# google-research/se3ds

Hardware: AMD Instinct MI355X
Metric: panoramas/sec (G+D train step) at 512x1024 RGB-D (higher is better)
Workload: dtype bf16; 1 GPU; configs/highres 512x1024 full GAN step train_g_d (G+D+hinge+depth+wc losses, clip, Adam, EMA), ResNet-101 gen_dims 128, per-GPU batch 8, d_step_per_g_step 1; per_gpu_batch=8, global_batch=8, parallelism=dp1

## Files before the change

se3ds_amd/csrc/conv.hip:

```cpp
#include <stdlib.h>

#include <cmath>
#include <type_traits>
#include "common.h"

namespace se3ds {
namespace {

typedef __attribute__((ext_vector_type(8))) __bf16 bf16x8_t;
typedef __attribute__((ext_vector_type(4))) short s16x4_t;
typedef __attribute__((ext_vector_type(16))) float f32x16_t;

constexpr int BM = 128;
constexpr int BN = 128;
constexpr int kThreads = 256;
constexpr int ROWB = 64;
constexpr int TILE_BYTES = 128 * ROWB;

enum { MODE_FWD = 0, MODE_DGRAD = 1 };

template <typename T> struct TT;
template <> struct TT<float> {
  static constexpr int EPC = 4;
  static constexpr int BK = 16;
// ... 1562 lines not shown
    constexpr int P = decltype(par_c)::value;
    unsigned char* xc = P ? xb1 : xb0;
    unsigned char* xn = P ? xb0 : xb1;
#define SE3DS_TAP(T_)                                                                      \
    k_step(std::integral_constant<int, T_>(),                                              \
           wsel(WST == 2 ? ((T_ + P) & 1) : (T_ % 3)),                                     \
           wsel(WST == 2 ? ((T_ + P + 1) & 1) : ((T_ + 2) % 3)), xc, xn, slab, next_slab)
    SE3DS_TAP(0); SE3DS_TAP(1); SE3DS_TAP(2); SE3DS_TAP(3); SE3DS_TAP(4);
    SE3DS_TAP(5); SE3DS_TAP(6); SE3DS_TAP(7); SE3DS_TAP(8);
#undef SE3DS_TAP
  };
  auto slab_even = [&](int slab, bool next_slab) {
    slab_body(std::integral_constant<int, 0>(), slab, next_slab);
  };
  auto slab_odd = [&](int slab, bool next_slab) {
    slab_body(std::integral_constant<int, 1>(), slab, next_slab);
  };
  for (int slab = 0; slab < nslabs; slab += 2) {
    slab_even(slab, slab + 1 < nslabs);
    if (slab + 1 < nslabs) slab_odd(slab + 1, slab + 2 < nslabs);
  }
  if (wm == 0) __builtin_amdgcn_s_barrier();

  int64_t opix[2];
#pragma unroll
  for (int j = 0; j < 2; ++j) {
    const int y = cur.y0 + wn * 2 + j, x = cur.x0 + l32;
    opix[j] = (y < p.oH && x < p.oW) ? ((int64_t)cur.img * p.oH + y) * p.oW + x : -1;
  }
  const int co_base = cur.n0 + wm * (CO / 2);
  const int opy0 = cur.y0, opx0 = cur.x0, opimg = cur.img;
  float* stats_row = ((MODE == MODE_FWD || BNB) && p.stats)
                         ? p.stats + ((int64_t)(cur.tile * 4 + wn) * 2) * p.oC : nullptr;
  constexpr bool LATE = M16 && CO == 256;
  bool have = false;
  auto next_item = [&]() {
    item += gridDim.x;
    have = item < nitems;
    if (have) {
      setup_item(item, cur, xptr, xmk, wbase);
      issue_prologue();
    }
  };
  if (!LATE) next_item();
  unsigned char* scratch = xb1 + wave * kEpiScratch<2>;
  if constexpr (M16) {
    int lane_e = lane;
    asm volatile("" : "+v"(lane_e));
    int64_t opix16[4];
#pragma unroll
    for (int j = 0; j < 4; ++j) {
      const int y = opy0 + wn * 2 + (j >> 1), x = opx0 + (j & 1) * 16 + (lane_e & 15);
      opix16[j] = (y < p.oH && x < p.oW) ? ((int64_t)opimg * p.oH + y) * p.oW + x : -1;
    }
    store_wave_lds16<BNB, false, CO == 128>(p, *reinterpret_cast<f32x4_t(*)[4][4]>(&acc16[0]), opix16, co_base,
                                            lane_e, scratch, stats_row);
    if (CO == 256)
      store_wave_lds16<BNB>(p, *reinterpret_cast<f32x4_t(*)[4][4]>(&acc16[CB16 - 4]), opix16,
                            co_base + 64, lane_e, scratch, stats_row);
  } else {
  store_wave_lds<2, BNB>(p, *reinterpret_cast<f32x16_t(*)[2][2]>(&acc[0]), opix, co_base, lane,
                         scratch, stats_row);
  if (NI == 4)
    store_wave_lds<2, BNB>(p, *reinterpret_cast<f32x16_t(*)[2][2]>(&acc[NI - 2]), opix, co_base + 64,
                           lane, scratch, stats_row);
  }
  if (LATE) next_item();
  if (!have) break;
  }
}


struct WgradParams {
  const void* x; int H, W, Cin;
  const void* dy; int Ho, Wo, Cout;
  int N, kh, kw, stride, pad_t, pad_l, wrap_w;
  const float* src_mask;
  int mask_binary;
  const float* row_scale;
  float* dw;
  int splits; int64_t l_per_split;
  int ci_tiles;
  int linear_k;
};

constexpr int WG_BL = 32;
constexpr int WG_ROWB_BF16 = 320;
constexpr int WG_ROWB_F32 = 528;

template <typename T>
__global__ void __launch_bounds__(kThreads, 2)
wgrad_kernel(const WgradParams p) {
  using tt = TT<T>;
  constexpr int ROWBYTES = sizeof(T) == 2 ? WG_ROWB_BF16 : WG_ROWB_F32;
  constexpr int TILE = WG_BL * ROWBYTES;
  __shared__ __attribute__((aligned(16))) unsigned char smem[2 * 2 * TILE];
  const int tid = threadIdx.x, lane = tid & 63, wave = tid >> 6;
  const int wm = wave >> 1, wn = wave & 1;
  const int tap = p.linear_k ? 0 : blockIdx.x / p.ci_tiles;
  const int ci0 = p.linear_k ? blockIdx.x * 128 : (blockIdx.x - tap * p.ci_tiles) * 128;
  const int co0 = blockIdx.y * 128;
  const int split = blockIdx.z;
  const int ky = tap / p.kw, kx = tap - ky * p.kw;
  const int Ktot = p.kh * p.kw * p.Cin;
  const int64_t L = (int64_t)p.N * p.Ho * p.Wo;
  const int64_t l_begin = (int64_t)split * p.l_per_split;
  int64_t l_end = l_begin + p.l_per_split;
  if (l_end > L) l_end = L;
  const int nsteps = l_begin < l_end ? (int)((l_end - l_begin + WG_BL - 1) / WG_BL) : 0;

  const T* __restrict__ x = (const T*)p.x;
  const T* __restrict__ dy = (const T*)p.dy;
  constexpr int EPC = tt::EPC;
  constexpr int CHUNKS_PER_ROW = 128 / EPC;
  constexpr int CH_PER_THREAD = WG_BL * CHUNKS_PER_ROW / kThreads;
  const bool vec_x = (p.Cin % EPC) == 0, vec_y = (p.Cout % EPC) == 0;

  uint4 rx[CH_PER_THREAD], ry[CH_PER_THREAD];

  int pn[CH_PER_THREAD], poy[CH_PER_THREAD], pox[CH_PER_THREAD];
#pragma unroll
  for (int q = 0; q < CH_PER_THREAD; ++q) {
    int id = tid + q * kThreads;
    int r = id / CHUNKS_PER_ROW;
    int64_t l = l_begin + r;
    if (l >= L) l = L - 1;
    pn[q] = (int)(l / ((int64_t)p.Ho * p.Wo));
    int rem = (int)(l - (int64_t)pn[q] * p.Ho * p.Wo);
    poy[q] = rem / p.Wo;
    pox[q] = rem - poy[q] * p.Wo;
  }

  auto load_step = [&](int st) {
#pragma unroll
    for (int q = 0; q < CH_PER_THREAD; ++q) {
      int id = tid + q * kThreads;
      int r = id / CHUNKS_PER_ROW, c = (id - r * CHUNKS_PER_ROW) * EPC;
      int64_t l = l_begin + (int64_t)st * WG_BL + r;
      T xe[EPC], ye[EPC];
#pragma unroll
      for (int e = 0; e < EPC; ++e) { xe[e] = tt::from_f(0.f); ye[e] = tt::from_f(0.f); }
      if (l < l_end && p.linear_k) {
        const int n = pn[q], oy = poy[q], ox = pox[q];
#pragma unroll
        for (int e = 0; e < EPC; ++e) {
          const int kk = ci0 + c + e;
          if (kk < Ktot) {
            const int t = kk / p.Cin, ci = kk - t * p.Cin;
            const int tky = t / p.kw, tkx = t - tky * p.kw;
            int sy = oy * p.stride - p.pad_t + tky, sx = ox * p.stride - p.pad_l + tkx;
            if (p.wrap_w) sx = sx < 0 ? sx + p.W : (sx >= p.W ? sx - p.W : sx);
            if ((unsigned)sy < (unsigned)p.H && (unsigned)sx < (unsigned)p.W) {
              const int64_t pix = ((int64_t)n * p.H + sy) * p.W + sx;
              float v = tt::to_f(x[pix * p.Cin + ci]);
              if (p.src_mask) v *= p.src_mask[pix];
              xe[e] = tt::from_f(v);
            }
          }
        }
      } else if (l < l_end) {
        const int n = pn[q], oy = poy[q], ox = pox[q];
        int sy = oy * p.stride - p.pad_t + ky, sx = ox * p.stride - p.pad_l + kx;
        if (p.wrap_w) sx = sx < 0 ? sx + p.W : (sx >= p.W ? sx - p.W : sx);
        if (sy >= 0 && sy < p.H && sx >= 0 && sx < p.W) {
          int64_t pix = ((int64_t)n * p.H + sy) * p.W + sx;
          const float mk = p.src_mask ? p.src_mask[pix] : 1.0f;
// ... 63 lines not shown
  for (int st = 0; st < nsteps; ++st) {
    const int stage = st & 1;
    if (st + 1 < nsteps) load_step(st + 1);
    const unsigned char* xt = smem + stage * 2 * TILE;
    const unsigned char* yt = xt + TILE;
    if (sizeof(T) == 2) {
      const int g16 = (lane >> 4) & 1, i16 = lane & 15;
      const int jrow = i16 >> 2, qcol = i16 & 3;
#pragma unroll
      for (int ks = 0; ks < 2; ++ks) {
        uint4 xf[2], yf[2];
#pragma unroll
        for (int t = 0; t < 2; ++t) {
          const int lb = ks * 16 + half * 8;
          const int xc = (wm * 64 + t * 32 + g16 * 16 + qcol * 4) * 2;
          const int yc = (wn * 64 + t * 32 + g16 * 16 + qcol * 4) * 2;
          s16x4_t x0 = __builtin_amdgcn_ds_read_tr16_b64_v4i16(
              (__attribute__((address_space(3))) s16x4_t*)(xt + (lb + jrow) * ROWBYTES + xc));
          s16x4_t x1 = __builtin_amdgcn_ds_read_tr16_b64_v4i16(
              (__attribute__((address_space(3))) s16x4_t*)(xt + (lb + 4 + jrow) * ROWBYTES + xc));
          s16x4_t y0 = __builtin_amdgcn_ds_read_tr16_b64_v4i16(
              (__attribute__((address_space(3))) s16x4_t*)(yt + (lb + jrow) * ROWBYTES + yc));
          s16x4_t y1 = __builtin_amdgcn_ds_read_tr16_b64_v4i16(
              (__attribute__((address_space(3))) s16x4_t*)(yt + (lb + 4 + jrow) * ROWBYTES + yc));
          uint2 a0 = __builtin_bit_cast(uint2, x0), a1 = __builtin_bit_cast(uint2, x1);
          uint2 b0 = __builtin_bit_cast(uint2, y0), b1 = __builtin_bit_cast(uint2, y1);
          xf[t] = make_uint4(a0.x, a0.y, a1.x, a1.y);
          yf[t] = make_uint4(b0.x, b0.y, b1.x, b1.y);
        }
#pragma unroll
        for (int i = 0; i < 2; ++i)
#pragma unroll
          for (int j = 0; j < 2; ++j)
            acc[i][j] = __builtin_amdgcn_mfma_f32_32x32x16_bf16(
                __builtin_bit_cast(bf16x8_t, yf[j]), __builtin_bit_cast(bf16x8_t, xf[i]),
                acc[i][j], 0, 0, 0);
      }
    } else {
#pragma unroll 4
      for (int k2 = 0; k2 < WG_BL / 2; ++k2) {
        const int l = k2 * 2 + half;
        float xa[2], yb[2];
#pragma unroll
        for (int t = 0; t < 2; ++t) {
          xa[t] = *reinterpret_cast<const float*>(xt + l * ROWBYTES + (wm * 64 + t * 32 + l32) * 4);
          yb[t] = *reinterpret_cast<const float*>(yt + l * ROWBYTES + (wn * 64 + t * 32 + l32) * 4);
        }
#pragma unroll
        for (int i = 0; i < 2; ++i)
#pragma unroll
          for (int j = 0; j < 2; ++j)
            acc[i][j] = __builtin_amdgcn_mfma_f32_32x32x2f32(yb[j], xa[i], acc[i][j], 0, 0, 0);
      }
    }
    if (st + 1 < nsteps) store_step(stage ^ 1);
    __syncthreads();
  }
  const int64_t K = (int64_t)p.kh * p.kw * p.Cin;
  float* __restrict__ dw = p.dw + (int64_t)split * K * p.Cout;
#pragma unroll
  for (int i = 0; i < 2; ++i) {
    const int ci = ci0 + wm * 64 + i * 32 + l32;
    if (ci >= (p.linear_k ? Ktot : p.Cin)) continue;
    float* row = dw + (p.linear_k ? (int64_t)ci : (int64_t)tap * p.Cin + ci) * p.Cout;
#pragma unroll
    for (int j = 0; j < 2; ++j)
#pragma unroll
      for (int g = 0; g < 4; ++g) {
        const int co = co0 + wn * 64 + j * 32 + g * 8 + half * 4;
        if (co + 3 < p.Cout && (p.Cout & 3) == 0) {
          *reinterpret_cast<float4*>(row + co) = make_float4(acc[i][j][g * 4], acc[i][j][g * 4 + 1],
                                                             acc[i][j][g * 4 + 2], acc[i][j][g * 4 + 3]);
        } else {
#pragma unroll
          for (int e = 0; e < 4; ++e)
            if (co + e < p.Cout) row[co + e] = acc[i][j][g * 4 + e];
        }
      }
  }
}

__device__ __attribute__((aligned(256))) unsigned char g_zero_page_w[512];

template <typename T>
__global__ void __launch_bounds__(kThreads, 2)
wgrad_glds_kernel(const WgradParams p) {
  using tt = TT<T>;
  constexpr int EPC = tt::EPC;
  constexpr int BL = sizeof(T) == 2 ? 64 : 32;
  constexpr int ROWBYTES = 128 * sizeof(T);
  constexpr int CPR = 128 / EPC;
  constexpr int RPI = 64 / CPR;
  constexpr int NI = BL / RPI / 4;
  constexpr int TILE = BL * ROWBYTES;
  __shared__ __attribute__((aligned(16))) unsigned char stage0[2 * TILE];
  __shared__ __attribute__((aligned(16))) unsigned char stage1[2 * TILE];
  const int tid = threadIdx.x, lane = tid & 63;
  const int wave = __builtin_amdgcn_readfirstlane(tid >> 6);
  const int wm = wave >> 1, wn = wave & 1;
  const int tap = blockIdx.x / p.ci_tiles;
  const int ci0 = (blockIdx.x - tap * p.ci_tiles) * 128;
  const int co0 = blockIdx.y * 128;
  const int split = blockIdx.z;
  const int ky = tap / p.kw, kx = tap - ky * p.kw;
  const int64_t L = (int64_t)p.N * p.Ho * p.Wo;
  const int64_t l_begin = (int64_t)split * p.l_per_split;
  int64_t l_end = l_begin + p.l_per_split;
  if (l_end > L) l_end = L;
  const int nsteps = l_begin < l_end ? (int)((l_end - l_begin + BL - 1) / BL) : 0;
  const T* __restrict__ x = (const T*)p.x;
  const T* __restrict__ dy = (const T*)p.dy;
  const T* zero = reinterpret_cast<const T*>(g_zero_page_w);

  int srow[NI], lch[NI];
  bool xc_ok[NI], yc_ok[NI];
  int pn[NI], poy[NI], pox[NI];
#pragma unroll
  for (int j = 0; j < NI; ++j) {
    srow[j] = (j * 4 + wave) * RPI + lane / CPR;
    const int pch = lane % CPR;
    lch[j] = sizeof(T) == 2 ? (pch ^ ((srow[j] & 3) << 2)) : pch;
    xc_ok[j] = ci0 + lch[j] * EPC + EPC <= p.Cin;
    yc_ok[j] = co0 + lch[j] * EPC + EPC <= p.Cout;
    int64_t l = l_begin + srow[j];
    if (l >= L) l = L - 1;
    pn[j] = (int)(l / ((int64_t)p.Ho * p.Wo));
    int rem = (int)(l - (int64_t)pn[j] * p.Ho * p.Wo);
    poy[j] = rem / p.Wo;
    pox[j] = rem - poy[j] * p.Wo;
  }

  const int dyoff = ky - p.pad_t, dxoff = kx - p.pad_l;
  const int st_ = p.stride;
  const int l_end_rel = (int)(l_end - l_begin);
  const bool lin = p.kh == 1 && p.kw == 1 && p.stride == 1 && p.pad_t == 0 && p.pad_l == 0;
  const int adv_y = BL / p.Wo, adv_x = BL - adv_y * p.Wo;
  int pixn[NI];
  bool okn[NI];
  float mnext[NI];
  auto look_ahead = [&](int st) {
#pragma unroll
    for (int j = 0; j < NI; ++j) {
      const int lrel = st * BL + srow[j];
      bool ok = xc_ok[j] && lrel < l_end_rel;
      int pix;
      if (lin) {
        pix = (int)l_begin + lrel;
      } else {
        int sy = poy[j] * st_ + dyoff, sx = pox[j] * st_ + dxoff;
        if (p.wrap_w) sx = sx < 0 ? sx + p.W : (sx >= p.W ? sx - p.W : sx);
        ok = ok && (unsigned)sy < (unsigned)p.H && (unsigned)sx < (unsigned)p.W;
        pix = (pn[j] * p.H + sy) * p.W + sx;
      }
      pixn[j] = pix;
      okn[j] = ok;
      mnext[j] = (p.src_mask && ok) ? p.src_mask[pix] : 1.0f;
    }
  };
  auto issue = [&](int st, unsigned char* xt) {
    unsigned char* yt = xt + TILE;
#pragma unroll
    for (int j = 0; j < NI; ++j) {
      const int lrel = st * BL + srow[j];
      const T* xs = zero + lch[j] * EPC;
      const T* ys = xs;
      if (okn[j] && mnext[j] != 0.0f) xs = x + (int64_t)pixn[j] * p.Cin + ci0 + lch[j] * EPC;
      if (yc_ok[j] && lrel < l_end_rel) ys = dy + (l_begin + lrel) * p.Cout + co0 + lch[j] * EPC;
      const int slab = (j * 4 + wave) * RPI * ROWBYTES;
      __builtin_amdgcn_global_load_lds((gas_ptr)xs, (las_ptr)(xt + slab), 16, 0, 0);
      __builtin_amdgcn_global_load_lds((gas_ptr)ys, (las_ptr)(yt + slab), 16, 0, 0);
      if (!lin) {
        pox[j] += adv_x;
        poy[j] += adv_y;
        if (pox[j] >= p.Wo) { pox[j] -= p.Wo; ++poy[j]; }
        if (poy[j] >= p.Ho) {
          const int t = poy[j] / p.Ho;
          pn[j] += t;
          poy[j] -= t * p.Ho;
        }
      }
    }
    look_ahead(st + 1);
  };

  f32x16_t acc[2][2];
#pragma unroll
  for (int i = 0; i < 2; ++i)
#pragma unroll
    for (int j = 0; j < 2; ++j)
#pragma unroll
      for (int r = 0; r < 16; ++r) acc[i][j][r] = 0.f;

  look_ahead(0);
  if (nsteps > 0) issue(0, stage0);
  __syncthreads();
  const int half = lane >> 5, l32 = lane & 31;
  auto l_step = [&](int st, unsigned char* cur, unsigned char* nxt) {
    if (st + 1 < nsteps) issue(st + 1, nxt);
    const unsigned char* xt = cur;
    const unsigned char* yt = xt + TILE;
    if (sizeof(T) == 2) {
      const int g16 = (lane >> 4) & 1, i16 = lane & 15;
      const int jrow = i16 >> 2, qcol = i16 & 3;
#pragma unroll
      for (int ks = 0; ks < BL / 16; ++ks) {
        uint4 xf[2], yf[2];
#pragma unroll
        for (int t = 0; t < 2; ++t) {
          const int lb = ks * 16 + half * 8;
          const int xcol = wm * 64 + t * 32 + g16 * 16 + qcol * 4;
          const int ycol = wn * 64 + t * 32 + g16 * 16 + qcol * 4;
          const int sw = (jrow & 3) << 2;
          const int xo = (((xcol >> 3) ^ sw) << 4) + ((xcol & 4) << 1);
          const int yo = (((ycol >> 3) ^ sw) << 4) + ((ycol & 4) << 1);
          s16x4_t x0 = __builtin_amdgcn_ds_read_tr16_b64_v4i16(
              (__attribute__((address_space(3))) s16x4_t*)(xt + (lb + jrow) * ROWBYTES + xo));
          s16x4_t x1 = __builtin_amdgcn_ds_read_tr16_b64_v4i16(
              (__attribute__((address_space(3))) s16x4_t*)(xt + (lb + 4 + jrow) * ROWBYTES + xo));
          s16x4_t y0 = __builtin_amdgcn_ds_read_tr16_b64_v4i16(
              (__attribute__((address_space(3))) s16x4_t*)(yt + (lb + jrow) * ROWBYTES + yo));
          s16x4_t y1 = __builtin_amdgcn_ds_read_tr16_b64_v4i16(
              (__attribute__((address_space(3))) s16x4_t*)(yt + (lb + 4 + jrow) * ROWBYTES + yo));
          uint2 a0 = __builtin_bit_cast(uint2, x0), a1 = __builtin_bit_cast(uint2, x1);
          uint2 b0 = __builtin_bit_cast(uint2, y0), b1 = __builtin_bit_cast(uint2, y1);
          xf[t] = make_uint4(a0.x, a0.y, a1.x, a1.y);
          yf[t] = make_uint4(b0.x, b0.y, b1.x, b1.y);
        }
#pragma unroll
        for (int i = 0; i < 2; ++i)
#pragma unroll
          for (int j = 0; j < 2; ++j)
            acc[i][j] = __builtin_amdgcn_mfma_f32_32x32x16_bf16(
                __builtin_bit_cast(bf16x8_t, yf[j]), __builtin_bit_cast(bf16x8_t, xf[i]),
                acc[i][j], 0, 0, 0);
      }
    } else {
#pragma unroll 4
      for (int k2 = 0; k2 < BL / 2; ++k2) {
        const int l = k2 * 2 + half;
        float xa[2], yb[2];
#pragma unroll
        for (int t = 0; t < 2; ++t) {
          xa[t] = *reinterpret_cast<const float*>(xt + l * ROWBYTES + (wm * 64 + t * 32 + l32) * 4);
          yb[t] = *reinterpret_cast<const float*>(yt + l * ROWBYTES + (wn * 64 + t * 32 + l32) * 4);
        }
#pragma unroll
        for (int i = 0; i < 2; ++i)
#pragma unroll
          for (int j = 0; j < 2; ++j)
            acc[i][j] = __builtin_amdgcn_mfma_f32_32x32x2f32(yb[j], xa[i], acc[i][j], 0, 0, 0);
      }
    }
    __syncthreads();
  };
  for (int st = 0; st < nsteps; st += 2) {
    l_step(st, stage0, stage1);
    if (st + 1 < nsteps) l_step(st + 1, stage1, stage0);
  }
  const int64_t K = (int64_t)p.kh * p.kw * p.Cin;
  float* __restrict__ dw = p.dw + (int64_t)split * K * p.Cout;
#pragma unroll
  for (int i = 0; i < 2; ++i) {
    const int ci = ci0 + wm * 64 + i * 32 + l32;
    if (ci >= p.Cin) continue;
    float* row = dw + ((int64_t)tap * p.Cin + ci) * p.Cout;
#pragma unroll
    for (int j = 0; j < 2; ++j)
#pragma unroll
      for (int g = 0; g < 4; ++g) {
        const int co = co0 + wn * 64 + j * 32 + g * 8 + half * 4;
        if (co + 3 < p.Cout && (p.Cout & 3) == 0) {
          *reinterpret_cast<float4*>(row + co) = make_float4(acc[i][j][g * 4], acc[i][j][g * 4 + 1],
                                                             acc[i][j][g * 4 + 2], acc[i][j][g * 4 + 3]);
        } else {
#pragma unroll
          for (int e = 0; e < 4; ++e)
            if (co + e < p.Cout) row[co + e] = acc[i][j][g * 4 + e];
        }
      }
  }
}

struct WgradTapsParams {
  const uint16_t* x; int H, W, Cin;
  const uint16_t* dy; int Ho, Wo, Cout;
  int N, pad_t, pad_l, wrap_w;
  const float* src_mask;
  float* dw;
  int steps_y, steps_x;
  int total_steps, steps_per_split;
  int dy_cstride, co_valid;
};

__global__ void __launch_bounds__(512)
wgrad_taps_kernel(const WgradTapsParams p) {
  typedef uint16_t T;
  constexpr int YROW = 256, XROW = 128, PC = 34;
  constexpr int YT = 64 * YROW;
  constexpr int XR = 4 * PC;
  constexpr int XPIECES = (XR + 7) / 8;
  constexpr int XT = XPIECES * 8 * XROW + 1024;
  constexpr int NST = 2;
  __shared__ __attribute__((aligned(16))) unsigned char stage0[YT + XT];
  __shared__ __attribute__((aligned(16))) unsigned char stage1[YT + XT];
  __shared__ __attribute__((aligned(16))) unsigned char stage2[NST == 3 ? YT + XT : 16];
  __shared__ __attribute__((aligned(16))) unsigned char sink[1024];
  const int tid = threadIdx.x, lane = tid & 63;
  const int wave = __builtin_amdgcn_readfirstlane(tid >> 6);
  const int iw = wave >> 2, cw = wave & 3;
  const int ci0 = blockIdx.x * 64, co0 = blockIdx.y * 128;
  const int split = blockIdx.z;
  const int st_begin = split * p.steps_per_split;
  int st_end = st_begin + p.steps_per_split;
  if (st_end > p.total_steps) st_end = p.total_steps;
  const int nsteps = st_end > st_begin ? st_end - st_begin : 0;
  const T* zero = reinterpret_cast<const T*>(g_zero_page_w);

  int ya[2], yb[2], ych[2];
#pragma unroll
  for (int j = 0; j < 2; ++j) {
    const int r = (wave * 2 + j) * 4 + (lane >> 4);
    ya[j] = r >> 5; yb[j] = r & 31;
    ych[j] = (lane & 15) ^ ((r & 3) << 2);
  }
  int xa[3], xb[3], xch[3];
#pragma unroll
  for (int j = 0; j < 3; ++j) {
    const int r = (wave + 8 * j) * 8 + (lane >> 3);
    xa[j] = r / PC; xb[j] = r - xa[j] * PC;
    if (r >= XR) xa[j] = 1 << 20;
    xch[j] = (lane & 7) ^ ((r & 2) << 1);
  }

  struct StepPos { int img, y0, x0; };
  auto step_pos = [&](int st) {
    int t = st_begin + st;
    StepPos sp;
    const int sx_i = t % p.steps_x; t /= p.steps_x;
    const int sy_i = t % p.steps_y;
    sp.img = t / p.steps_y;
    sp.y0 = sy_i * 2; sp.x0 = sx_i * 32;
// ... 1490 lines not shown
#pragma unroll
    for (int j = 0; j < 2; ++j) {
      const int cr = cr0 + 32 * j;
      const int c = c0 + cr;
      const int64_t k = k0 + kq;
      if (c < Cout && k < K) {
        uint16_t o[8];
#pragma unroll
        for (int e = 0; e < 8; ++e) o[e] = f32_to_bf16(tile[kq + e][cr]);
        *reinterpret_cast<uint4*>(wt + (int64_t)c * K + k) = *reinterpret_cast<const uint4*>(o);
      }
    }
  }
}

constexpr int kRouteRing = 8;
static thread_local int t_route_ring[kRouteRing];
static thread_local unsigned t_route_n = 0;

static thread_local int64_t* t_defer_row = nullptr;

static void launch_wgrad_reduce(const float* part, int splits, int64_t n, int accumulate,
                                const float* out_scale, float* out, hipStream_t s) {
  if (t_defer_row != nullptr && !accumulate && out_scale == nullptr && (n % 4) == 0 &&
      (((uintptr_t)part | (uintptr_t)out) & 15) == 0) {
    t_defer_row[0] = (int64_t)(uintptr_t)part;
    t_defer_row[1] = splits;
    t_defer_row[2] = n / 4;
    t_defer_row[3] = (int64_t)(uintptr_t)out;
    t_defer_row[4] = 1;
    t_defer_row = nullptr;
    return;
  }
  if ((n % 4) == 0 && (((uintptr_t)part | (uintptr_t)out) & 15) == 0)
    SE3DS_LAUNCH(wgrad_reduce_vec, wgrad_reduce_vec_kernel, dim3(grid_for(n / 4, 256)), dim3(256),
                 0, s, part, splits, n / 4, accumulate, out_scale, out);
  else
    SE3DS_LAUNCH(wgrad_reduce_scalar, wgrad_reduce_scalar_kernel, dim3(grid_for(n, 256)), dim3(256),
                 0, s, part, splits, n, accumulate, out_scale, out);
}

int fill_classes(IgemmParams& p, int mode, int bm = BM) {
  int total = 0;
  if (mode == MODE_FWD) {
    p.n_classes = 1;
    p.cls_py[0] = p.cls_px[0] = 0;
    p.cls_tile_start[0] = 0;
    int64_t m = (int64_t)p.N * p.oH * p.oW;
    total = (int)ceil_div(m, bm);
    p.cls_tile_start[1] = total;
    p.fd_hw[0] = make_fastdiv((uint32_t)(p.oH * p.oW));
    p.fd_w[0] = make_fastdiv((uint32_t)p.oW);
    return total;
  }
  const int s = p.stride;
  p.n_classes = s * s;
  int c = 0;
  for (int py = 0; py < s; ++py)
    for (int px = 0; px < s; ++px, ++c) {
      p.cls_py[c] = py; p.cls_px[c] = px;
      p.cls_tile_start[c] = total;
      int cH = (p.oH - py + s - 1) / s, cW = (p.oW - px + s - 1) / s;
      if (cH < 0) cH = 0;
      if (cW < 0) cW = 0;
      p.fd_hw[c] = make_fastdiv((uint32_t)(cH * cW));
      p.fd_w[c] = make_fastdiv((uint32_t)cW);
      total += (int)ceil_div((int64_t)p.N * cH * cW, bm);
    }
  p.cls_tile_start[c] = total;
  return total;
}

}

void note_conv_route(int route) { t_route_ring[t_route_n++ % kRouteRing] = route; }

}

using namespace se3ds;


static bool thin_on() { return getenv("SE3DS_NO_THIN") == nullptr; }

static int big_tile_mode() {
  const char* e = getenv("SE3DS_BIG_TILE");
  return e ? atoi(e) : -1;
}

static int halo_tile_channels(const IgemmParams& p) {
  const char* e = getenv("SE3DS_HALO_TILE");
  const int mode = e ? atoi(e) : -1;
  if (mode == 0) return 0;
  if ((p.oC % 128) != 0) return 0;
  if (mode == 128 || (p.oC % 256) != 0) return 128;
  if (mode == 256) return 256;
  const int64_t tiles = (int64_t)p.N * ceil_div(p.oH, 8) * ceil_div(p.oW, 32);
  const int64_t items256 = tiles * (p.oC / 256);
  const double eff256 = (double)items256 / (double)(ceil_div(items256, (int64_t)256) * 256);
  const int64_t items128 = items256 * 2;
  const double eff128 = 0.85 * (double)items128 / (double)(ceil_div(items128, (int64_t)256) * 256);
  return eff256 >= eff128 ? 256 : 128;
}

static bool halo_m16() {
  const char* e = getenv("SE3DS_HALO_M16");
  return e ? atoi(e) != 0 : true;
}

static int big_tile_channels(const IgemmParams& p, int mode) {
  const int g_big_tile = big_tile_mode();
  if (g_big_tile == 0) return 0;
  const int co = (p.oC % 256) == 0 ? 256 : ((p.oC % 128) == 0 ? 128 : 0);
  if (!co) return 0;
  if (g_big_tile == 1) return co;
  int64_t m = 0;
  const int s = mode == MODE_FWD ? 1 : p.stride;
  for (int py = 0; py < s; ++py)
    for (int px = 0; px < s; ++px)
      m += (int64_t)p.N * ((p.oH - py + s - 1) / s) * ((p.oW - px + s - 1) / s);
  const double kCus = 256.0;
  const double big_items = (double)ceil_div(m, (int64_t)256) * (p.oC / co);
  const double small_items = (double)ceil_div(m, (int64_t)128) * ceil_div(p.oC, 128);
  if (co != 256) return 0;
  const double gain = 1.25;
  const double t_small = std::ceil(small_items / (2 * kCus)) * 2.0;
  const double t_big = std::ceil(big_items / kCus) * (co == 256 ? 4.0 : 2.0) / gain;
  return t_big < t_small ? co : 0;
}

static int64_t fwd_stats_rows(const IgemmParams& p, int dtype, int stride, int kh, int kw,
                              bool glds, int mode = MODE_FWD) {
  if (!glds || dtype != SE3DS_BF16) return 0;
  if (mode == MODE_DGRAD && stride != 1) return 0;
  const int64_t M = (int64_t)p.N * p.oH * p.oW;
  if (stride == 1 && kh == 3 && kw == 3 && halo_tile_channels(p))
    return (int64_t)p.N * ceil_div(p.oH, 8) * ceil_div(p.oW, 32) * 4;
  if (big_tile_channels(p, mode)) return ceil_div(M, (int64_t)256) * 4;
  if ((p.oC % BN) == 0) return ceil_div(M, (int64_t)BM) * (BM / 64);
  return 0;
}

extern "C" {

static int conv_common(int mode, const void* src, const void* w, void* out, int dtype, int n,
                       int h, int wdt, int cin, int ho, int wo, int cout, int kh, int kw,
                       int stride, int pad_t, int pad_l, int wrap_w, const float* src_mask,
                       int mask_binary, const float* scale, const float* bias, const float* row_a,
                       const float* row_b, int act, float act_alpha, void* stream,
                       float* stats = nullptr, const void* addend = nullptr,
                       const void* bn_x = nullptr, const uint8_t* bn_mask = nullptr,
                       const float* bn_mean = nullptr, const float* bn_rstd = nullptr,
                       int bn_act = 0, float bn_alpha = 0.f, int64_t o_pitch = 0, int64_t o_off = 0,
                       int bias_mod = 0) {
  if (n <= 0 || h <= 0 || wdt <= 0 || cin <= 0 || ho <= 0 || wo <= 0 || cout <= 0 || kh <= 0 ||
      kw <= 0 || stride <= 0 || stride > 2)
    return SE3DS_E_BADSHAPE;
  if (wrap_w && mode == MODE_DGRAD && (stride != 1 || wo != wdt)) return SE3DS_E_UNSUPPORTED;
  if (dtype != SE3DS_F32 && dtype != SE3DS_BF16) return SE3DS_E_BADDTYPE;
  if ((int64_t)n * h * wdt >= ((int64_t)1 << 31) || (int64_t)n * ho * wo >= ((int64_t)1 << 31))
    return SE3DS_E_BADSHAPE;
  IgemmParams p;
  p.src = src; p.w = w; p.out = out;
  p.N = n; p.kh = kh; p.kw = kw; p.stride = stride; p.pad_t = pad_t; p.pad_l = pad_l;
  p.wrap_w = wrap_w; p.src_mask = src_mask; p.mask_binary = mask_binary; p.scale = scale;
  p.bias = bias; p.row_a = row_a;
  p.row_b = row_b; p.act = act; p.act_alpha = act_alpha;
  const int bk = dtype == SE3DS_F32 ? 16 : 32;
  const int64_t K = (int64_t)kh * kw * cin;
  if (mode == MODE_FWD) {
    p.sH = h; p.sW = wdt; p.sC = cin; p.oH = ho; p.oW = wo; p.oC = cout;
    p.w_tap = cin; p.w_n = K;
  } else {
    p.sH = ho; p.sW = wo; p.sC = cout; p.oH = h; p.oW = wdt; p.oC = cin;
    p.w_tap = (int64_t)cin * cout; p.w_n = cout;
  }
  p.vec = (p.sC % bk) == 0;
  p.o_pitch = o_pitch > 0 ? o_pitch : p.oW;
  p.o_off = o_off;
  p.bias_mod = bias_mod;
  const bool pitched = o_pitch > 0 || bias_mod > 0;
#ifdef SE3DS_PROBE
  { const char* e = getenv("SE3DS_PROBE_MODE"); p.probe = e ? atoi(e) : 0; }
#endif
  p.stats = nullptr;
  p.addend = addend;
  hipStream_t s = as_stream(stream);
  const bool glds = (p.sC % (2 * bk)) == 0 && (src_mask == nullptr || mask_binary);
  if (stats != nullptr && !(fwd_stats_rows(p, dtype, stride, kh, kw, glds, mode) > 0))
    return SE3DS_E_UNSUPPORTED;
  if (stats != nullptr && mode == MODE_DGRAD &&
      (bn_x == nullptr || bn_mean == nullptr || bn_rstd == nullptr || (p.oC & 7) != 0))
    return SE3DS_E_UNSUPPORTED;
  p.stats = stats;
  p.bn_x = (mode == MODE_DGRAD && stats != nullptr) ? (const uint16_t*)bn_x : nullptr;
  p.bn_mask = bn_mask; p.bn_mean = bn_mean; p.bn_rstd = bn_rstd;
  p.bn_act = bn_act; p.bn_alpha = bn_alpha;
  if (mode == MODE_DGRAD && dtype == SE3DS_BF16 && kh == 4 && kw == 4 && stride == 2 && cin <= 4 &&
      cout == 128 && src_mask == nullptr && row_a == nullptr && bias == nullptr && act == 0 &&
      !wrap_w && (pad_t == 0 || pad_t == 2) && (pad_l == 0 || pad_l == 2) &&
      thin_on()) {
    int64_t blocks = (int64_t)p.N * ceil_div(p.oH, kThinSRows) * ceil_div(p.oW, kThinSCols);
    if (blocks > 2 * 256) blocks = 2 * 256;
    SE3DS_LAUNCH(thin_s2_dgrad, thin_s2_dgrad_kernel, dim3((unsigned)blocks), dim3(256), 0, s, p);
    return check_launch("conv2d_dgrad(thin s2)");
  }
  if (mode == MODE_FWD && dtype == SE3DS_BF16 && cin <= kThinCinMax && (cout % 128) == 0 &&
      kh * kw * cin <= kThinKMax && kh <= 7 && kw <= 7 && stats == nullptr && addend == nullptr &&
      !pitched && thin_on()) {
    const ThinCinLds L = thin_cin_lds(kh, kw, cin, stride);
    static size_t lds_set = 0;
    if (L.bytes > lds_set) {
      if (hipFuncSetAttribute((const void*)thin_cin_fwd_kernel,
                              hipFuncAttributeMaxDynamicSharedMemorySize, (int)L.bytes) != hipSuccess)
        return SE3DS_E_LAUNCH;
      lds_set = L.bytes;
    }
    int64_t blocks = (int64_t)p.N * ceil_div(p.oH, kThinFRows) * ceil_div(p.oW, kThinCols);
    const int64_t resident = 256;
    if (blocks > resident) blocks = resident;
    SE3DS_LAUNCH(thin_cin_fwd, thin_cin_fwd_kernel, dim3((unsigned)blocks), dim3(kThinFThreads),
                 L.bytes, s, p);
    return check_launch("conv2d_fwd(thin cin)");
  }
  if (mode == MODE_DGRAD && dtype == SE3DS_BF16 && kh == 3 && kw == 3 && stride == 1 && cout <= 4 &&
      (cin % 64) == 0 && cin <= kThinDCinMax && src_mask == nullptr && row_a == nullptr &&
      thin_on()) {
    int64_t blocks = (int64_t)p.N * ceil_div(p.oH, kThinDRows) * ceil_div(p.oW, kThinCols);
    if (blocks > 2 * 256) blocks = 2 * 256;
    SE3DS_LAUNCH(thin_cout_dgrad, thin_cout_dgrad_kernel, dim3((unsigned)blocks), dim3(256), 0, s, p);
    return check_launch("conv2d_dgrad(thin)");
  }
  if (mode == MODE_FWD && dtype == SE3DS_BF16 && kh == 3 && kw == 3 && stride == 1 && cout <= 4 &&
      (cin % 64) == 0 && cin <= 128 && src_mask == nullptr && row_a == nullptr &&
      stats == nullptr && addend == nullptr && thin_on()) {
    const size_t lds = thin_lds_bytes(cin, cout);
    static size_t lds_set = 0;
    if (lds > lds_set) {
      if (hipFuncSetAttribute((const void*)thin_cout_fwd_kernel,
                              hipFuncAttributeMaxDynamicSharedMemorySize, (int)lds) != hipSuccess)
        return SE3DS_E_LAUNCH;
      lds_set = lds;
    }
    int64_t blocks = (int64_t)p.N * ceil_div(p.oH, kThinRows) * ceil_div(p.oW, kThinCols);
    if (blocks > 2 * 256) blocks = 2 * 256;
    SE3DS_LAUNCH(thin_cout_fwd, thin_cout_fwd_kernel, dim3((unsigned)blocks), dim3(256), lds, s, p);
    return check_launch("conv2d_fwd(thin)");
  }
  if (glds && dtype == SE3DS_BF16 && stride == 1 && kh == 3 && kw == 3) {
    const int co = halo_tile_channels(p);
    if (co) {
      p.halo_ty = ceil_div(p.oH, 8);
      p.halo_tx = ceil_div(p.oW, 32);
      const int64_t items = (int64_t)p.N * p.halo_ty * p.halo_tx * (p.oC / co);
      dim3 grid((unsigned)(items < 256 ? items : 256));
      if (co == 256 && halo_m16()) {
        if (mode == MODE_FWD) SE3DS_LAUNCH(halo256_fwd_m16, (igemm_halo_kernel<MODE_FWD, 256, 2, false, true>), grid, dim3(512), 0, s, p);
        else if (p.bn_x) SE3DS_LAUNCH(halo256_dgrad_bn_m16, (igemm_halo_kernel<MODE_DGRAD, 256, 2, true, true>), grid, dim3(512), 0, s, p);
        else SE3DS_LAUNCH(halo256_dgrad_m16, (igemm_halo_kernel<MODE_DGRAD, 256, 2, false, true>), grid, dim3(512), 0, s, p);
      } else if (co == 256) {
        if (mode == MODE_FWD) SE3DS_LAUNCH(halo256_fwd_m32, (igemm_halo_kernel<MODE_FWD, 256, 2>), grid, dim3(512), 0, s, p);
        else if (p.bn_x) SE3DS_LAUNCH(halo256_dgrad_bn_m32, (igemm_halo_kernel<MODE_DGRAD, 256, 2, true>), grid, dim3(512), 0, s, p);
        else SE3DS_LAUNCH(halo256_dgrad_m32, (igemm_halo_kernel<MODE_DGRAD, 256, 2>), grid, dim3(512), 0, s, p);
      } else {
        if (halo_m16()) {
          if (mode == MODE_FWD) SE3DS_LAUNCH(halo128_fwd_m16, (igemm_halo_kernel<MODE_FWD, 128, 3, false, true>), grid, dim3(512), 0, s, p);
// ... 211 lines not shown
    bytes = bytes > thin ? bytes : thin;
  }
  return bytes > taps_bytes ? bytes : taps_bytes;
}

int se3ds_conv2d_wgrad(const void* x, const void* dy, float* dw, int dtype, int n, int h, int w,
                       int cin, int ho, int wo, int cout, int kh, int kw, int stride, int pad_t,
                       int pad_l, int wrap_w, const float* in_mask, int in_mask_binary,
                       const float* row_scale, const float* out_scale, int accumulate,
                       void* workspace, size_t workspace_bytes, void* stream) {
  if (n <= 0 || h <= 0 || w <= 0 || cin <= 0 || ho <= 0 || wo <= 0 || cout <= 0 || kh <= 0 ||
      kw <= 0 || stride <= 0)
    return SE3DS_E_BADSHAPE;
  if (dtype != SE3DS_F32 && dtype != SE3DS_BF16) return SE3DS_E_BADDTYPE;
  if (workspace_bytes < se3ds_conv2d_wgrad_workspace_bytes(n, ho, wo, cin, cout, kh, kw))
    return SE3DS_E_WORKSPACE;
  hipStream_t s = as_stream(stream);
  if (dtype == SE3DS_BF16 && stride == 1 && row_scale == nullptr &&
      (in_mask == nullptr || in_mask_binary)) {
    int tsteps = 0;
    const int tsplits = wgrad_taps_splits(n, ho, wo, cin, cout, kh, kw, &tsteps);
    if (tsplits > 0) {
      WgradTapsParams q;
      q.x = (const uint16_t*)x; q.H = h; q.W = w; q.Cin = cin;
      q.dy = (const uint16_t*)dy; q.Ho = ho; q.Wo = wo; q.Cout = cout;
      q.N = n; q.pad_t = pad_t; q.pad_l = pad_l; q.wrap_w = wrap_w; q.src_mask = in_mask;
      q.dw = (float*)workspace;
      q.steps_y = ceil_div(ho, 2); q.steps_x = ceil_div(wo, 32);
      q.total_steps = tsteps;
      q.steps_per_split = ceil_div(tsteps, tsplits);
      q.dy_cstride = cout; q.co_valid = cout;
      dim3 tgrid((unsigned)(cin / 64), (unsigned)(cout / 128), (unsigned)tsplits);
      if (!wrap_w)
        if (halo_m16()) SE3DS_LAUNCH(wgrad_taps3_m16, wgrad_taps3_kernel<true>, tgrid, dim3(512), 0, s, q);
        else SE3DS_LAUNCH(wgrad_taps3_m32, wgrad_taps3_kernel<false>, tgrid, dim3(512), 0, s, q);
      else
        SE3DS_LAUNCH(wgrad_taps_wrap, wgrad_taps_kernel, tgrid, dim3(512), 0, s, q);
      const int64_t tnel = (int64_t)9 * cin * cout;
      launch_wgrad_reduce((const float*)workspace, tsplits, tnel, accumulate, out_scale, dw, s);
      return check_launch("conv2d_wgrad(taps)");
    }
  }
  if (dtype == SE3DS_BF16 && stride <= 2 && thin_cin_wgrad_ok(cin, cout, kh, kw)) {
    ThinCinWgradParams q;
    q.x = (const uint16_t*)x; q.dy = (const uint16_t*)dy; q.part = (float*)workspace;
    q.N = n; q.H = h; q.W = w; q.Cin = cin; q.Ho = ho; q.Wo = wo; q.Cout = cout; q.kh = kh;
    q.kw = kw; q.stride = stride; q.pad_t = pad_t; q.pad_l = pad_l; q.wrap_w = wrap_w;
    q.src_mask = in_mask; q.row_scale = row_scale;
    const size_t lds = thin_cin_wgrad_lds(kh, kw, cin, stride);
    static size_t lds_set = 0;
    if (lds > lds_set) {
      if (hipFuncSetAttribute((const void*)thin_cin_wgrad_kernel,
                              hipFuncAttributeMaxDynamicSharedMemorySize, (int)lds) != hipSuccess)
        return SE3DS_E_LAUNCH;
      lds_set = lds;
    }
    int64_t blocks = (int64_t)n * ceil_div(ho, kThinWRows) * ceil_div(wo, kThinCols);
    if (blocks > 256) blocks = 256;
    SE3DS_LAUNCH(thin_cin_wgrad, thin_cin_wgrad_kernel, dim3((unsigned)blocks), dim3(kThinWThreads), lds, s, q);
    const int64_t tnel = (int64_t)kh * kw * cin * cout;
    launch_wgrad_reduce((const float*)workspace, (int)blocks, tnel, accumulate, out_scale, dw, s);
    return check_launch("conv2d_wgrad(thin cin)");
  }
  WgradParams p;
  p.x = x; p.H = h; p.W = w; p.Cin = cin; p.dy = dy; p.Ho = ho; p.Wo = wo; p.Cout = cout;
  p.N = n; p.kh = kh; p.kw = kw; p.stride = stride; p.pad_t = pad_t; p.pad_l = pad_l;
  p.wrap_w = wrap_w; p.src_mask = in_mask; p.mask_binary = in_mask_binary; p.row_scale = row_scale;
  p.dw = (float*)workspace;
  p.ci_tiles = (int)ceil_div(cin, 128);
  p.linear_k = cin <= 16 ? 1 : 0;
  const int64_t L = (int64_t)n * ho * wo;
  const int64_t row_tiles = p.linear_k ? ceil_div((int64_t)kh * kw * cin, 128)
                                       : (int64_t)kh * kw * p.ci_tiles;
  const int64_t tiles = row_tiles * ceil_div(cout, 128);
  p.splits = wgrad_splits(L, tiles, (int64_t)kh * kw * cin * cout);
  p.l_per_split = ceil_div(ceil_div(L, p.splits), WG_BL) * WG_BL;
  dim3 grid((unsigned)row_tiles, (unsigned)ceil_div(cout, 128), (unsigned)p.splits);
  const int epc = dtype == SE3DS_F32 ? 4 : 8;
  const bool glds = !p.linear_k && (in_mask == nullptr || in_mask_binary) &&
                    row_scale == nullptr &&
                    (cin % epc) == 0 && (cout % epc) == 0;
  if (glds) {
    p.l_per_split = ceil_div(ceil_div(L, p.splits), 64) * 64;
    if (dtype == SE3DS_F32) SE3DS_LAUNCH(wgrad_glds_f32, wgrad_glds_kernel<float>, grid, dim3(kThreads), 0, s, p);
    else SE3DS_LAUNCH(wgrad_glds_bf16, wgrad_glds_kernel<uint16_t>, grid, dim3(kThreads), 0, s, p);
  } else if (dtype == SE3DS_F32) {
    SE3DS_LAUNCH(wgrad_f32, wgrad_kernel<float>, grid, dim3(kThreads), 0, s, p);
  } else {
    SE3DS_LAUNCH(wgrad_bf16, wgrad_kernel<uint16_t>, grid, dim3(kThreads), 0, s, p);
  }
  const int64_t nel = (int64_t)kh * kw * cin * cout;
  launch_wgrad_reduce((const float*)workspace, p.splits, nel, accumulate, out_scale, dw, s);
  return check_launch("conv2d_wgrad");
}

int se3ds_conv2d_wgrad_partial(const void* x, const void* dy, float* dw, int dtype, int n, int h,
                               int w, int cin, int ho, int wo, int cout, int kh, int kw, int stride,
                               int pad_t, int pad_l, int wrap_w, const float* in_mask,
                               int in_mask_binary, const float* row_scale, void* workspace,
                               size_t workspace_bytes, int64_t* reduce_row, void* stream) {
  if (reduce_row == nullptr) return SE3DS_E_BADSHAPE;
  reduce_row[4] = 0;
  t_defer_row = reduce_row;
  const int rc = se3ds_conv2d_wgrad(x, dy, dw, dtype, n, h, w, cin, ho, wo, cout, kh, kw, stride,
                                    pad_t, pad_l, wrap_w, in_mask, in_mask_binary, row_scale,
                                    nullptr, 0, workspace, workspace_bytes, stream);
  t_defer_row = nullptr;
  return rc;
}

int se3ds_wgrad_reduce_multi(const int64_t* table, int rows, int64_t workgroups, void* stream) {
  if (rows <= 0 || workgroups <= 0) return SE3DS_OK;
  if (workgroups >= ((int64_t)1 << 31)) return SE3DS_E_BADSHAPE;
  SE3DS_LAUNCH(wgrad_reduce_multi, wgrad_reduce_multi_kernel, dim3((unsigned)workgroups), dim3(256),
               0, as_stream(stream), table, rows);
  return check_launch("wgrad_reduce_multi");
}

int se3ds_wgrad_reduce_tile(void) { return kRedTile; }

uint32_t se3ds_fastdiv_host(uint32_t n, uint32_t d) {
  const FastDiv f = make_fastdiv(d);
  const uint32_t t = (uint32_t)(((uint64_t)n * f.m) >> 32);
  return (t + ((n - t) >> f.s1)) >> f.s2;
}

static int wgrad_taps_thin_splits(int n, int h, int w, int cin, int cout, int k, int* steps) {
  if (k != 3 || cout > 8 || (cin % 64) != 0) return 0;
  const int64_t total = (int64_t)n * ceil_div(h, 2) * ceil_div(w, 32);
  if (total > (1 << 30)) return 0;
  *steps = (int)total;
  const int64_t tiles = cin / 64;
  int64_t sp = ceil_div((int64_t)256, tiles);
  if (sp > total / 8) sp = total / 8;
  if (sp < 1) sp = 1;
  return (int)sp;
}

size_t se3ds_conv2d_wgrad_swapped_workspace_bytes(int n, int h, int w, int cin, int cout, int k) {
  const size_t a = se3ds_conv2d_wgrad_workspace_bytes(n, h, w, cout, cin, k, k) +
                   sizeof(float) * (size_t)k * k * cin * cout + 64;
  int steps = 0;
  const int sp = wgrad_taps_thin_splits(n, h, w, cin, cout, k, &steps);
  const size_t b = sp ? (size_t)n * h * w * 16 + 256 + sizeof(float) * (size_t)sp * 9 * cin * cout + 64
                      : 0;
  const size_t c = (k == 3 && cout <= 4) ? sizeof(float) * (size_t)kThinQSlabs * 9 * cin * cout + 64 : 0;
  const size_t ab = a > b ? a : b;
  return ab > c ? ab : c;
}

int se3ds_conv2d_wgrad_swapped(const void* x, const void* dy, float* dw, int dtype, int n, int h,
                               int w, int cin, int cout, int k, int pad, int accumulate,
                               void* workspace, size_t workspace_bytes, void* stream) {
  if (workspace_bytes < se3ds_conv2d_wgrad_swapped_workspace_bytes(n, h, w, cin, cout, k))
    return SE3DS_E_WORKSPACE;
  if (dtype == SE3DS_BF16 && k == 3 && cout <= 4 && (cin % 32) == 0 && cin <= 128 &&
      workspace_bytes >= sizeof(float) * (size_t)kThinQSlabs * 9 * cin * cout &&
      thin_on()) {
    hipStream_t s = as_stream(stream);
    ThinCoutWgradParams q;
    q.x = (const uint16_t*)x; q.dy = (const uint16_t*)dy; q.part = (float*)workspace;
    q.N = n; q.H = h; q.W = w; q.Cin = cin; q.Cout = cout; q.pad = pad;
    const size_t lds = thin_cout_wgrad_lds(cin);
    int64_t blocks = (int64_t)n * ceil_div(h, kThinQRows) * ceil_div(w, kThinCols);
    if (blocks > kThinQSlabs) blocks = kThinQSlabs;
    const int tiles_per_wave = ceil_div(9 * (cin / 32), 8);
#define SE3DS_THIN_CW(M)                                                                          \
  do {                                                                                            \
// ... 96 lines not shown
```

Before: 41.81 panoramas/sec.

## Specialize wgrad glds kernel on linear/mask and pipeline mask prefetch with counted waits

Templates the bf16 weight-gradient global-to-LDS kernel on whether the conv is 1x1 linear and whether a source mask is present. It replaces per-row index arrays with incremental pointer strides and issues the mask loads asynchronously one step ahead. It also swaps __syncthreads for explicit vmcnt waits plus s_barrier, with an optional 3-stage variant reachable only through probe builds. The aim is to cut address arithmetic and the serialized mask-load latency in the main loop, at the cost of inline-asm waitcnt assumptions that are fragile to compiler scheduling.

```diff
diff --git a/se3ds_amd/csrc/conv.hip b/se3ds_amd/csrc/conv.hip
--- a/se3ds_amd/csrc/conv.hip
+++ b/se3ds_amd/csrc/conv.hip
@@ -1668,6 +1668,9 @@
   int splits; int64_t l_per_split;
   int ci_tiles;
   int linear_k;
+#ifdef SE3DS_PROBE
+  int probe;
+#endif
 };
 
 constexpr int WG_BL = 32;
@@ -1897,8 +1900,14 @@
 
 __device__ __attribute__((aligned(256))) unsigned char g_zero_page_w[512];
 
-template <typename T>
-__global__ void __launch_bounds__(kThreads, 2)
+__device__ __forceinline__ float gload_f32_async(const float* src) {
+  float v;
+  asm volatile("global_load_dword %0, %1, off" : "=v"(v) : "v"(src) : "memory");
+  return v;
+}
+
+template <typename T, bool LIN, bool MASK, int NST>
+__global__ void __launch_bounds__(kThreads, NST == 2 ? 2 : 1)
 wgrad_glds_kernel(const WgradParams p) {
   using tt = TT<T>;
   constexpr int EPC = tt::EPC;
@@ -1907,9 +1916,17 @@
   constexpr int CPR = 128 / EPC;
   constexpr int RPI = 64 / CPR;
   constexpr int NI = BL / RPI / 4;
+  constexpr int SROWS = 4 * RPI;
   constexpr int TILE = BL * ROWBYTES;
-  __shared__ __attribute__((aligned(16))) unsigned char stage0[2 * TILE];
-  __shared__ __attribute__((aligned(16))) unsigned char stage1[2 * TILE];
+  constexpr int STAGE = 2 * TILE;
+  static_assert(NST == 2 || NST == 3, "two or three stages");
+  static_assert(NI == 4, "the counted wait assumes 2 * NI = 8 transfers per wave and step");
+  __shared__ __attribute__((aligned(16))) unsigned char smem[NST * STAGE];
+#ifdef SE3DS_PROBE
+  const int probe = p.probe;
+#else
+  constexpr int probe = 0;
+#endif
   const int tid = threadIdx.x, lane = tid & 63;
   const int wave = __builtin_amdgcn_readfirstlane(tid >> 6);
   const int wm = wave >> 1, wn = wave & 1;
@@ -1923,68 +1940,60 @@
   int64_t l_end = l_begin + p.l_per_split;
   if (l_end > L) l_end = L;
   const int nsteps = l_begin < l_end ? (int)((l_end - l_begin + BL - 1) / BL) : 0;
-  const T* __restrict__ x = (const T*)p.x;
-  const T* __restrict__ dy = (const T*)p.dy;
-  const T* zero = reinterpret_cast<const T*>(g_zero_page_w);
-
-  int srow[NI], lch[NI];
-  bool xc_ok[NI], yc_ok[NI];
-  int pn[NI], poy[NI], pox[NI];
-#pragma unroll
-  for (int j = 0; j < NI; ++j) {
-    srow[j] = (j * 4 + wave) * RPI + lane / CPR;
-    const int pch = lane % CPR;
-    lch[j] = sizeof(T) == 2 ? (pch ^ ((srow[j] & 3) << 2)) : pch;
-    xc_ok[j] = ci0 + lch[j] * EPC + EPC <= p.Cin;
-    yc_ok[j] = co0 + lch[j] * EPC + EPC <= p.Cout;
-    int64_t l = l_begin + srow[j];
-    if (l >= L) l = L - 1;
-    pn[j] = (int)(l / ((int64_t)p.Ho * p.Wo));
-    int rem = (int)(l - (int64_t)pn[j] * p.Ho * p.Wo);
-    poy[j] = rem / p.Wo;
-    pox[j] = rem - poy[j] * p.Wo;
-  }
+  const int l_end_rel = l_begin < l_end ? (int)(l_end - l_begin) : 0;
+
+  const int row0 = wave * RPI + lane / CPR;
+  const int pch = lane % CPR;
+  const int lch = sizeof(T) == 2 ? (pch ^ ((row0 & 3) << 2)) : pch;
+  const bool xc_ok = ci0 + lch * EPC + EPC <= p.Cin;
+  const bool yc_ok = co0 + lch * EPC + EPC <= p.Cout;
+  const unsigned char* const zp = g_zero_page_w + lch * 16;
+  const unsigned char* yp =
+      yc_ok ? reinterpret_cast<const unsigned char*>((const T*)p.dy + (l_begin + row0) * p.Cout + co0 + lch * EPC)
+            : zp;
+  const uint32_t yslot = yc_ok ? (uint32_t)(SROWS * sizeof(T)) * (uint32_t)p.Cout : 0u;
+  const uint32_t ystep = yc_ok ? (uint32_t)(BL * sizeof(T)) * (uint32_t)p.Cout : 0u;
+  const unsigned char* xp =
+      !xc_ok ? zp
+             : reinterpret_cast<const unsigned char*>(
+                   (const T*)p.x + (LIN ? (l_begin + row0) * p.Cin : (int64_t)0) + ci0 + lch * EPC);
+  const uint32_t cinb = (uint32_t)sizeof(T) * (uint32_t)p.Cin;
+  const uint32_t xslot = LIN && xc_ok ? (uint32_t)SROWS * cinb : 0u;
+  const uint32_t xstep = LIN && xc_ok ? (uint32_t)BL * cinb : 0u;
 
   const int dyoff = ky - p.pad_t, dxoff = kx - p.pad_l;
   const int st_ = p.stride;
-  const int l_end_rel = (int)(l_end - l_begin);
-  const bool lin = p.kh == 1 && p.kw == 1 && p.stride == 1 && p.pad_t == 0 && p.pad_l == 0;
   const int adv_y = BL / p.Wo, adv_x = BL - adv_y * p.Wo;
-  int pixn[NI];
-  bool okn[NI];
-  float mnext[NI];
-  auto look_ahead = [&](int st) {
+  int pn[NI], poy[NI], pox[NI];
+  if (!LIN) {
 #pragma unroll
     for (int j = 0; j < NI; ++j) {
-      const int lrel = st * BL + srow[j];
-      bool ok = xc_ok[j] && lrel < l_end_rel;
-      int pix;
-      if (lin) {
-        pix = (int)l_begin + lrel;
+      int64_t l = l_begin + row0 + j * SROWS;
+      if (l >= L) l = L - 1;
+      pn[j] = (int)(l / ((int64_t)p.Ho * p.Wo));
+      int rem = (int)(l - (int64_t)pn[j] * p.Ho * p.Wo);
+      poy[j] = rem / p.Wo;
+      pox[j] = rem - poy[j] * p.Wo;
+    }
+  }
+  int pixn[NI], pix2[NI];
+  bool okn[NI], ok2[NI];
+  float mcur[NI], mnew[NI];
+#pragma unroll
+  for (int j = 0; j < NI; ++j) { pixn[j] = pix2[j] = 0; okn[j] = ok2[j] = false; mcur[j] = mnew[j] = 1.0f; }
+  auto prefetch = [&](int s) {
+#pragma unroll
+    for (int j = 0; j < NI; ++j) {
+      const int lrel = s * BL + row0 + j * SROWS;
+      if (LIN) {
+        if (MASK) mnew[j] = gload_f32_async(p.src_mask + (lrel < l_end_rel ? l_begin + lrel : (int64_t)0));
       } else {
         int sy = poy[j] * st_ + dyoff, sx = pox[j] * st_ + dxoff;
         if (p.wrap_w) sx = sx < 0 ? sx + p.W : (sx >= p.W ? sx - p.W : sx);
-        ok = ok && (unsigned)sy < (unsigned)p.H && (unsigned)sx < (unsigned)p.W;
-        pix = (pn[j] * p.H + sy) * p.W + sx;
-      }
-      pixn[j] = pix;
-      okn[j] = ok;
-      mnext[j] = (p.src_mask && ok) ? p.src_mask[pix] : 1.0f;
-    }
-  };
-  auto issue = [&](int st, unsigned char* xt) {
-    unsigned char* yt = xt + TILE;
-#pragma unroll
-    for (int j = 0; j < NI; ++j) {
-      const int lrel = st * BL + srow[j];
-      const T* xs = zero + lch[j] * EPC;
-      const T* ys = xs;
-      if (okn[j] && mnext[j] != 0.0f) xs = x + (int64_t)pixn[j] * p.Cin + ci0 + lch[j] * EPC;
-      if (yc_ok[j] && lrel < l_end_rel) ys = dy + (l_begin + lrel) * p.Cout + co0 + lch[j] * EPC;
-      const int slab = (j * 4 + wave) * RPI * ROWBYTES;
-      __builtin_amdgcn_global_load_lds((gas_ptr)xs, (las_ptr)(xt + slab), 16, 0, 0);
-      __builtin_amdgcn_global_load_lds((gas_ptr)ys, (las_ptr)(yt + slab), 16, 0, 0);
-      if (!lin) {
+        const bool ok = xc_ok && lrel < l_end_rel && (unsigned)sy < (unsigned)p.H && (unsigned)sx < (unsigned)p.W;
+        ok2[j] = ok;
+        pix2[j] = ok ? (pn[j] * p.H + sy) * p.W + sx : 0;
+        if (MASK) mnew[j] = gload_f32_async(p.src_mask + pix2[j]);
         pox[j] += adv_x;
         poy[j] += adv_y;
         if (pox[j] >= p.Wo) { pox[j] -= p.Wo; ++poy[j]; }
@@ -1995,7 +2004,48 @@
         }
       }
     }
-    look_ahead(st + 1);
+  };
+  auto wait_commit = [&](bool deep) {
+    if (probe == 3) deep = false;
+    if (MASK) {
+#define SE3DS_WGRAD_COMMIT(WAIT)                                                                       \
+  asm volatile(WAIT "\n\tv_mov_b32 %0, %4\n\tv_mov_b32 %1, %5\n\tv_mov_b32 %2, %6\n\tv_mov_b32 %3, %7"   \
+               : "=&v"(mcur[0]), "=&v"(mcur[1]), "=&v"(mcur[2]), "=&v"(mcur[3])                        \
+               : "v"(mnew[0]), "v"(mnew[1]), "v"(mnew[2]), "v"(mnew[3]) : "memory")
+      if (deep) SE3DS_WGRAD_COMMIT("s_waitcnt vmcnt(8) lgkmcnt(0)");
+      else SE3DS_WGRAD_COMMIT("s_waitcnt vmcnt(0) lgkmcnt(0)");
+#undef SE3DS_WGRAD_COMMIT
+    } else {
+      if (deep) asm volatile("s_waitcnt vmcnt(8) lgkmcnt(0)" ::: "memory");
+      else asm volatile("s_waitcnt vmcnt(0) lgkmcnt(0)" ::: "memory");
+    }
+#pragma unroll
+    for (int j = 0; j < NI; ++j) { pixn[j] = pix2[j]; okn[j] = ok2[j]; }
+  };
+  auto issue = [&](int s, int stage, const bool full) {
+    unsigned char* xt = smem + stage * STAGE;
+    unsigned char* yt = xt + TILE;
+#pragma unroll
+    for (int j = 0; j < NI; ++j) {
+      const bool rok = full || s * BL + row0 + j * SROWS < l_end_rel;
+      bool xok = LIN ? rok : okn[j];
+      if (MASK) xok = xok && mcur[j] != 0.0f;
+      const unsigned char* xs = LIN ? xp + j * xslot : xp + (uint64_t)(uint32_t)pixn[j] * cinb;
+      const unsigned char* ys = yp + j * yslot;
+      if (!(LIN && !MASK && full)) xs = xok ? xs : zp;
+      if (!full) ys = rok ? ys : zp;
+      const int slab = (j * 4 + wave) * RPI * ROWBYTES;
+      if (probe != 3) {
+        glds16(xs, xt + slab);
+        glds16(ys, yt + slab);
+      }
+    }
+    xp += xstep;
+    yp += ystep;
+  };
+  auto issue_any = [&](int s, int stage) {
+    if (s < nsteps - 1) issue(s, stage, true);
+    else issue(s, stage, false);
   };
 
   f32x16_t acc[2][2];
@@ -2006,15 +2056,27 @@
 #pragma unroll
       for (int r = 0; r < 16; ++r) acc[i][j][r] = 0.f;
 
-  look_ahead(0);
-  if (nsteps > 0) issue(0, stage0);
-  __syncthreads();
+  prefetch(0);
+  wait_commit(false);
+#pragma unroll
+  for (int s = 0; s < NST - 1; ++s) {
+    prefetch(s + 1);
+    if (s < nsteps) issue_any(s, s);
+    wait_commit(NST == 3 && s < nsteps);
+  }
+  asm volatile("" ::: "memory");
+  __builtin_amdgcn_s_barrier();
+  asm volatile("" ::: "memory");
   const int half = lane >> 5, l32 = lane & 31;
-  auto l_step = [&](int st, unsigned char* cur, unsigned char* nxt) {
-    if (st + 1 < nsteps) issue(st + 1, nxt);
-    const unsigned char* xt = cur;
+  auto l_step = [&](int st, int cur_stage, int far_stage) {
+    const int s = st + NST - 1;
+    const bool issued = s < nsteps;
+    prefetch(s + 1);
+    if (issued) issue_any(s, far_stage);
+    const unsigned char* xt = smem + cur_stage * STAGE;
     const unsigned char* yt = xt + TILE;
-    if (sizeof(T) == 2) {
+    if (probe == 2) {
+    } else if (sizeof(T) == 2) {
       const int g16 = (lane >> 4) & 1, i16 = lane & 15;
       const int jrow = i16 >> 2, qcol = i16 & 3;
 #pragma unroll
@@ -2066,12 +2128,24 @@
             acc[i][j] = __builtin_amdgcn_mfma_f32_32x32x2f32(yb[j], xa[i], acc[i][j], 0, 0, 0);
       }
     }
-    __syncthreads();
-  };
-  for (int st = 0; st < nsteps; st += 2) {
-    l_step(st, stage0, stage1);
-    if (st + 1 < nsteps) l_step(st + 1, stage1, stage0);
-  }
+    wait_commit(NST == 3 && issued);
+    asm volatile("" ::: "memory");
+    __builtin_amdgcn_s_barrier();
+    asm volatile("" ::: "memory");
+  };
+  if (NST == 3) {
+    for (int st = 0; st < nsteps; st += 3) {
+      l_step(st, 0, 2);
+      if (st + 1 < nsteps) l_step(st + 1, 1, 0);
+      if (st + 2 < nsteps) l_step(st + 2, 2, 1);
+    }
+  } else {
+    for (int st = 0; st < nsteps; st += 2) {
+      l_step(st, 0, 1);
+      if (st + 1 < nsteps) l_step(st + 1, 1, 0);
+    }
+  }
+  if (probe == 1) return;
   const int64_t K = (int64_t)p.kh * p.kw * p.Cin;
   float* __restrict__ dw = p.dw + (int64_t)split * K * p.Cout;
 #pragma unroll
@@ -3728,6 +3802,25 @@
 
 static bool thin_on() { return getenv("SE3DS_NO_THIN") == nullptr; }
 
+#ifdef SE3DS_PROBE
+static int probe_mode() {
+  const char* e = getenv("SE3DS_PROBE_MODE");
+  return e ? atoi(e) : 0;
+}
+#endif
+
+constexpr int kWgradGldsStages = 2;
+template <int NST>
+static void launch_wgrad_glds_bf16(bool lin, bool masked, dim3 grid, hipStream_t s, const WgradParams& p) {
+  if (lin) {
+    if (masked) SE3DS_LAUNCH(wgrad_glds_bf16, (wgrad_glds_kernel<uint16_t, true, true, NST>), grid, dim3(kThreads), 0, s, p);
+    else SE3DS_LAUNCH(wgrad_glds_bf16, (wgrad_glds_kernel<uint16_t, true, false, NST>), grid, dim3(kThreads), 0, s, p);
+  } else {
+    if (masked) SE3DS_LAUNCH(wgrad_glds_bf16, (wgrad_glds_kernel<uint16_t, false, true, NST>), grid, dim3(kThreads), 0, s, p);
+    else SE3DS_LAUNCH(wgrad_glds_bf16, (wgrad_glds_kernel<uint16_t, false, false, NST>), grid, dim3(kThreads), 0, s, p);
+  }
+}
+
 static int big_tile_mode() {
   const char* e = getenv("SE3DS_BIG_TILE");
   return e ? atoi(e) : -1;
@@ -3826,7 +3919,7 @@
   p.bias_mod = bias_mod;
   const bool pitched = o_pitch > 0 || bias_mod > 0;
 #ifdef SE3DS_PROBE
-  { const char* e = getenv("SE3DS_PROBE_MODE"); p.probe = e ? atoi(e) : 0; }
+  p.probe = probe_mode();
 #endif
   p.stats = nullptr;
   p.addend = addend;
@@ -4204,8 +4297,22 @@
                     (cin % epc) == 0 && (cout % epc) == 0;
   if (glds) {
     p.l_per_split = ceil_div(ceil_div(L, p.splits), 64) * 64;
-    if (dtype == SE3DS_F32) SE3DS_LAUNCH(wgrad_glds_f32, wgrad_glds_kernel<float>, grid, dim3(kThreads), 0, s, p);
-    else SE3DS_LAUNCH(wgrad_glds_bf16, wgrad_glds_kernel<uint16_t>, grid, dim3(kThreads), 0, s, p);
+    const bool lin = kh == 1 && kw == 1 && stride == 1 && pad_t == 0 && pad_l == 0;
+    const bool masked = in_mask != nullptr;
+    if (dtype == SE3DS_F32) {
+      if (masked) SE3DS_LAUNCH(wgrad_glds_f32, (wgrad_glds_kernel<float, false, true, 2>), grid, dim3(kThreads), 0, s, p);
+      else SE3DS_LAUNCH(wgrad_glds_f32, (wgrad_glds_kernel<float, false, false, 2>), grid, dim3(kThreads), 0, s, p);
+    } else {
+      int nst = kWgradGldsStages;
+#ifdef SE3DS_PROBE
+      p.probe = probe_mode() % 10;
+      if (probe_mode() >= 10) nst = 5 - nst;
+#endif
+      if (nst == kWgradGldsStages) launch_wgrad_glds_bf16<kWgradGldsStages>(lin, masked, grid, s, p);
+#ifdef SE3DS_PROBE
+      else launch_wgrad_glds_bf16<5 - kWgradGldsStages>(lin, masked, grid, s, p);
+#endif
+    }
   } else if (dtype == SE3DS_F32) {
     SE3DS_LAUNCH(wgrad_f32, wgrad_kernel<float>, grid, dim3(kThreads), 0, s, p);
   } else {
```

After: 41.73 panoramas/sec. Within noise of the previous version (-0.2%).
